# isteiakakis/Homomorphic-Encryption-Algorithms-Diploma-Thesis

Measured on AMD Instinct MI355X. Metric: CKKS matvec ciphertexts/sec (N=2^15, L=10), higher is better.
Workload: dtype u64; 1 GPU; he_linalg BatchedMatrix::matmul diag x col, 4096x4096 ct x ct matvec, N=2^15, L=10, default Galois keys; batch_per_gpu=128, n=4096, key_switches_per_matvec=18204, parallelism=replicated matrix+keys, dp1 over input vectors, batch_global=128

## Files before the change

### homomorphic-encryption-algorithms-diploma-thesis_amd/csrc/hec_engine.hip

```cpp
#include <algorithm>
#include <cmath>
#include <complex>
#include <cstdio>
#include <cstdlib>
#include <cstring>
#include <exception>
#include <limits>
#include <mutex>
#include <set>
#include <thread>
#include <tuple>

#include "hec_internal.h"

#include <dlfcn.h>
#include <unistd.h>
#include <rccl/rccl.h>
#include "hecdna.h"

using namespace hec;
using u128 = unsigned __int128;

struct HecComm {
    virtual ~HecComm() = default;
// ... 390 lines not shown
        fan_divide_round(c, ACC + l * N, 2 * (l + 1) * N, (l + 1) * N, Z, B * ng, 2, l, (int)c.K - 1);
    }
    for (int q = 0; q < ng; ++q) {
        ProfScope k(c, "k:k_ntt/divround_b", (6.0 + in_nk) * B * l);
        divide_round(c, ACC + q * sacc + l * N, 2 * (l + 1) * N, (l + 1) * N,
                     PolyArr{ACC + q * sacc, 2 * (l + 1) * N, (l + 1) * N}, IN, in_nk, OUT[q], B, 2, l, (int)c.K - 1,
                     c.p_inv.data(), c.p_inv_q.data(), Z + q * sz, elts[q], 2);
    }
}

void keyswitch(Ctx &c, Scratch &s, PolyArr T, const u64 *key, PolyArr IN, int in_nk, PolyArr OUT, int B, int l,
               u32 elt = 1)
{
    const u64 N = c.N;
    const std::size_t top = s.top;
    u64 *D = s.take(B * l * N), *E = s.take((u64)B * (l + 1) * l * N), *ACC = s.take((u64)B * 2 * (l + 1) * N),
        *Z = s.take((u64)B * 2 * l * N);
    int pmap[HEC_MAXL + 1];
    for (int i = 0; i <= HEC_MAXL; ++i) pmap[i] = i;
    const bool fan = c.fan_out && c.fused_modup_mac;
    const double K = l + 1;
    {
        ProfScope ps(c, "ks_intt");
        ProfScope k(c, fan ? "k:k_ntt/intt_b" : "k:k_ntt/intt2", 2.0 * B * l, fan ? 1 : 2);
        ntt_strided(c, true, T.p, T.sb, D, l * N, l, pmap, B * l, elt, fan ? 1 : 3);
    }
    if (c.fused_modup_mac) {
        {
            ProfScope ps(c, "ks_modup_a");
            ProfScope k(c, fan ? "k:k_fan2j/modup" : "k:k_ntt/modup_a", (double)B * l * (l + 1), 1);
            if (fan) fan_modup(c, D, E, B, l);
            else ks_modup_mac(c, D, E, T, key, ACC, B, l, 1, elt);
        }
        {
            ProfScope ps(c, "ks_bmac");
            ProfScope k(c, "k:k_bmac", (double)B * l * l + (double)B * l + 2.0 * l * K + 2.0 * B * K,
                        1);
            ks_modup_mac(c, D, E, T, key, ACC, B, l, 2, elt);
        }
    } else {
        {
            ProfScope ps(c, "ks_modup");
            ks_modup(c, D, E, B, l);
        }
        {
            ProfScope ps(c, "ks_mac");
            ks_mac(c, T, E, key, ACC, B, l, elt);
        }
    }
    moddown(c, ACC, Z, IN, in_nk, OUT, B, l, elt);
    s.top = top;
}

constexpr int HOIST_GROUP = 6;
struct Hoist {
    u64 *D = nullptr, *E = nullptr;
    int *zl = nullptr;
    u64 *acc0 = nullptr;
    u64 sacc = 0;
    u64 *acc(int q) const { return acc0 + (u64)q * sacc; }
};
std::size_t hoist_words(const Ctx &c, std::size_t B, std::size_t l)
{
    return c.N * B * (l + (l + 1) * l + (std::size_t)HOIST_GROUP * 2 * (l + 1)) +
           ((1 + B * l * (HEC_ZCAP + 1)) * sizeof(int) + 7) / 8 + 4 * 64;
}
// ... 818 lines not shown
        for (uint64_t i = 0; i < count; ++i) {
            need(bit_sizes[i] >= 2 && bit_sizes[i] <= 60, "bit_sizes is invalid");
            ++cnt[bit_sizes[i]];
        }
        const u64 factor = 2 * N;
        std::map<int, std::vector<u64>> table;
        for (auto &[b, k] : cnt) {
            u64 v = (((u64)1 << b) - 1) / factor * factor + 1;
            const u64 lo = (u64)1 << (b - 1);
            std::size_t left = k;
            while (left && v > lo) {
                if (isprime(v)) { table[b].push_back(v); --left; }
                v -= factor;
            }
            if (left) throw std::logic_error("failed to find enough qualifying primes");
        }
        for (uint64_t i = 0; i < count; ++i) {
            out[i] = table[bit_sizes[i]].back();
            table[bit_sizes[i]].pop_back();
        }
    });
}

int hec_context_create(uint64_t N, const uint64_t *mod, uint64_t K, int device, hec_context **out)
{
    return guard([&] {
        need(out != nullptr, "out is null");
        need(N >= 1024 && N <= 65536 && !(N & (N - 1)), "poly_modulus_degree must be a power of two in [2^10, 2^16]");
        need(K >= 2 && K - 1 <= HEC_MAXL, "coeff_modulus size is invalid");
        for (uint64_t i = 0; i < K; ++i)
            need(isprime(mod[i]) && (mod[i] - 1) % (2 * N) == 0 && !(mod[i] >> 60), "coeff_modulus is invalid");
        for (uint64_t i = 0; i < K; ++i)
            for (uint64_t j = 0; j < i; ++j) need(mod[i] != mod[j], "coeff_modulus is invalid");
        HEC_HIP(hipSetDevice(device));
        auto *ctx = new hec_context();
        Ctx &c = ctx->c;
        c.device = device;
        if (const char *f = std::getenv("HEC_FUSED_MODUP_MAC")) c.fused_modup_mac = f[0] != '0';
        if (const char *f = std::getenv("HEC_FUSE_GALOIS")) c.fuse_galois = f[0] != '0';
        if (const char *f = std::getenv("HEC_FAN")) c.fan_out = f[0] != '0';
        if (const char *f = std::getenv("HEC_HOIST_SCAN")) c.hoist_scan = std::atoi(f);
        if (const char *f = std::getenv("HEC_LANES")) c.lanes = std::max(1, std::atoi(f));
        if (const char *f = std::getenv("HEC_HOIST")) c.hoist = f[0] != '0';
        if (const char *f = std::getenv("HEC_HMAC")) c.hmac_cfg = std::atoi(f);
        if (const char *f = std::getenv("HEC_HMAC_ODD3")) c.hmac_odd3 = std::atoi(f);
        if (const char *f = std::getenv("HEC_HOIST_MIN")) c.hoist_min_children = std::max(1, std::atoi(f));
        if (const char *f = std::getenv("HEC_TENSOR_DEFER")) c.tensor_defer_max = std::max(1, std::atoi(f));
        if (const char *f = std::getenv("HEC_TENSOR_BUFS")) c.tensor_defer_bufs = std::max(1, std::atoi(f));
        if (const char *f = std::getenv("HEC_TENSOR_XCD")) c.tensor_xcd = std::max(0, std::atoi(f));
        if (const char *f = std::getenv("HEC_POISON")) c.poison = f[0] != '0';
        if (const char *f = std::getenv("HEC_LANE_SERIAL")) c.lane_serial = f[0] != '0';
        if (const char *f = std::getenv("HEC_DEBUG_LANES")) c.debug_lanes = f[0] != '0';
        if (const char *f = std::getenv("HEC_KERNEL_MEMOPS")) c.kernel_memops = f[0] != '0';
        if (const char *f = std::getenv("HEC_SPLIT_BFLY")) c.split_bfly = std::atoi(f);
        if (const char *f = std::getenv("HEC_NTTB_SHFL")) c.nttb_shfl = std::min(2, std::max(0, std::atoi(f)));
        if (const char *f = std::getenv("HEC_NTTB_SHFL_DR")) c.nttb_shfl_dr = std::atoi(f) != 0;
        if (const char *f = std::getenv("HEC_HMAC_INT")) c.hmac_int = std::atoi(f) != 0;
        if (const char *f = std::getenv("HEC_MODDOWN1")) c.moddown1 = std::atoi(f) != 0;
        if (const char *f = std::getenv("HEC_NT_E")) c.nt_e = std::atoi(f) != 0;
        if (const char *f = std::getenv("HEC_BMAC_SPLIT")) c.bmac_split = f[0] != '0';
        c.N = N;
        c.logN = __builtin_ctzll(N);
        c.K = K;
        c.L = K - 1;
        c.q.assign(mod, mod + K);
        for (u64 q : c.q) c.bits.push_back(64 - __builtin_clzll(q));
        HEC_HIP(hipStreamCreateWithFlags(&c.stream, hipStreamNonBlocking));
        c.own_stream = true;
        std::vector<ulonglong2> tw(K * N), itw(K * N);
        std::vector<u64> psipow(K * 2 * N);
// ... 46 lines not shown
            for (std::size_t k = 0; k < v.size(); ++k) r[k] = (double)v[k].x;
            return r;
        };
        const std::vector<double> twf = to_d(tw), itwf = to_d(itw), twbf = to_d(twb), itwbf = to_d(itwb);
        for (auto [dst, src] : {std::pair{&c.twf, &twf}, std::pair{&c.itwf, &itwf}, std::pair{&c.twbf, &twbf},
                                std::pair{&c.itwbf, &itwbf}}) {
            HEC_HIP(hipMalloc(dst, K * N * sizeof(double)));
            HEC_HIP(hipMemcpy(*dst, src->data(), K * N * sizeof(double), hipMemcpyHostToDevice));
        }
        HEC_HIP(hipMalloc(&c.twb, K * N * sizeof(ulonglong2)));
        HEC_HIP(hipMalloc(&c.itwb, K * N * sizeof(ulonglong2)));
        HEC_HIP(hipMemcpy(c.twb, twb.data(), K * N * sizeof(ulonglong2), hipMemcpyHostToDevice));
        HEC_HIP(hipMemcpy(c.itwb, itwb.data(), K * N * sizeof(ulonglong2), hipMemcpyHostToDevice));
        {
            std::vector<u64> tba(K * N, 0);
            for (uint64_t i = 0; i < K; ++i)
                if (!c.hprimes[i].fp)
                    for (uint64_t k = 0; k < N; ++k) tba[i * N + k] = (u64)(((u128)twb[i * N + k].x << 31) % c.q[i]);
            HEC_HIP(hipMalloc(&c.twbs, K * N * sizeof(u64)));
            HEC_HIP(hipMemcpy(c.twbs, tba.data(), K * N * sizeof(u64), hipMemcpyHostToDevice));
        }
        {
            HEC_HIP(hipMalloc(&c.psipow, psipow.size() * sizeof(u64)));
            HEC_HIP(hipMemcpy(c.psipow, psipow.data(), psipow.size() * sizeof(u64), hipMemcpyHostToDevice));
            std::vector<u64> cji(c.L * K);
            for (std::size_t J = 0; J < c.L; ++J)
                for (std::size_t I = 0; I < K; ++I) cji[J * K + I] = c.q[J] % c.q[I];
            HEC_HIP(hipMalloc(&c.cji, cji.size() * sizeof(u64)));
            HEC_HIP(hipMemcpy(c.cji, cji.data(), cji.size() * sizeof(u64), hipMemcpyHostToDevice));
            HEC_HIP(hipMalloc(&c.zflag, 2 * sizeof(int)));
            HEC_HIP(hipMemset(c.zflag, 0, 2 * sizeof(int)));
        }
        {
            std::vector<int> tab((c.L + 1) * (HEC_MAXL + 2), 0);
            c.imap_nint.assign(c.L + 1, 0);
            for (std::size_t l = 1; l <= c.L; ++l) {
                int *t = tab.data() + l * (HEC_MAXL + 2), n = 0;
                for (int pass = 0; pass < 2; ++pass)
                    for (int I = 0; I <= (int)l; ++I) {
                        const int kI = I == (int)l ? (int)K - 1 : I;
                        const bool fp = c.hprimes[kI].fp != 0;
                        if ((pass == 0) != fp) t[n++] = I;
                    }
                for (int I = 0; I <= (int)l; ++I)
                    if (!c.hprimes[I == (int)l ? K - 1 : I].fp) ++c.imap_nint[l];
            }
            HEC_HIP(hipMalloc(&c.imap, tab.size() * sizeof(int)));
            HEC_HIP(hipMemcpy(c.imap, tab.data(), tab.size() * sizeof(int), hipMemcpyHostToDevice));
        }
        HEC_HIP(hipMalloc(&c.primes, K * sizeof(DevPrime)));
        HEC_HIP(hipMemcpy(c.primes, c.hprimes.data(), K * sizeof(DevPrime), hipMemcpyHostToDevice));
        HEC_HIP(hipMalloc(&c.tw, K * N * sizeof(ulonglong2)));
        HEC_HIP(hipMalloc(&c.itw, K * N * sizeof(ulonglong2)));
        HEC_HIP(hipMemcpy(c.tw, tw.data(), K * N * sizeof(ulonglong2), hipMemcpyHostToDevice));
        HEC_HIP(hipMemcpy(c.itw, itw.data(), K * N * sizeof(ulonglong2), hipMemcpyHostToDevice));
        {
            std::vector<u64> ta(K * N, 0), ita(K * N, 0);
            for (uint64_t i = 0; i < K; ++i) {
                if (c.hprimes[i].fp) continue;
                const u64 q = c.q[i];
                for (uint64_t k = 0; k < N; ++k) {
                    ta[i * N + k] = (u64)(((u128)tw[i * N + k].x << 31) % q);
                    ita[i * N + k] = (u64)(((u128)itw[i * N + k].x << 31) % q);
                }
            }
            HEC_HIP(hipMalloc(&c.tws, K * N * sizeof(u64)));
            HEC_HIP(hipMalloc(&c.itws, K * N * sizeof(u64)));
            HEC_HIP(hipMemcpy(c.tws, ta.data(), K * N * sizeof(u64), hipMemcpyHostToDevice));
            HEC_HIP(hipMemcpy(c.itws, ita.data(), K * N * sizeof(u64), hipMemcpyHostToDevice));
        }
        const u64 P = c.q[K - 1];
        for (uint64_t i = 0; i < c.L; ++i) {
            const u64 q = c.q[i], pi = invm(P % q, q);
            c.p_inv.push_back(pi);
            c.p_inv_q.push_back(shoupq(pi, q));
// ... 60 lines not shown
            c.own_stream = false;
        } else {
            HEC_HIP(hipStreamCreateWithFlags(&c.stream, hipStreamNonBlocking));
            c.own_stream = true;
        }
    });
}

int hec_context_set_option(hec_context *ctx, const char *name, int64_t value)
{
    return guard([&] {
        need(ctx && name, "null argument");
        set_device(ctx);
        const std::string n(name);
        auto in = [&](int64_t lo, int64_t hi) {
            if (value < lo || value > hi)
                throw std::invalid_argument("option " + n + " takes " + std::to_string(lo) + ".." + std::to_string(hi));
            return (int)value;
        };
        auto apply = [&](Ctx &c) {
            if (n == "lanes") c.lanes = (int)std::max<int64_t>(1, value);
            else if (n == "lane_min_batch") c.lane_min_batch = (int)std::max<int64_t>(1, value);
            else if (n == "poison") c.poison = value != 0;
            else if (n == "lane_serial") c.lane_serial = value != 0;
            else if (n == "debug_lanes") c.debug_lanes = value != 0;
            else if (n == "kernel_memops") c.kernel_memops = value != 0;
            else if (n == "split_bfly") c.split_bfly = in(0, 4);
            else if (n == "nttb_shfl") c.nttb_shfl = in(0, 2);
            else if (n == "nttb_shfl_dr") c.nttb_shfl_dr = in(0, 1);
            else if (n == "hmac_int") c.hmac_int = in(0, 1);
            else if (n == "moddown1") c.moddown1 = in(0, 1);
            else if (n == "nt_e") c.nt_e = in(0, 1);
            else if (n == "bmac_split") c.bmac_split = value != 0;
            else if (n == "hoist") c.hoist = value != 0;
            else if (n == "hoist_min") c.hoist_min_children = (int)std::max<int64_t>(1, value);
            else if (n == "hmac") c.hmac_cfg = in(0, 2);
            else if (n == "hmac_odd3") c.hmac_odd3 = in(0, 1);
            else if (n == "hoist_scan") c.hoist_scan = in(0, 1);
            else if (n == "fan") c.fan_out = value != 0;
            else if (n == "fuse_galois") c.fuse_galois = value != 0;
            else if (n == "fused_modup_mac") c.fused_modup_mac = value != 0;
            else if (n == "tensor_defer") c.tensor_defer_max = (int)std::max<int64_t>(1, value);
            else if (n == "tensor_bufs") c.tensor_defer_bufs = (int)std::max<int64_t>(1, value);
            else if (n == "tensor_xcd") c.tensor_xcd = (int)std::max<int64_t>(0, value);
            else throw std::invalid_argument("unknown option");
        };
        HEC_HIP(hipStreamSynchronize(ctx->c.stream));
        apply(ctx->c);
        for (hec_context *l : ctx->lanes) {
            HEC_HIP(hipStreamSynchronize(l->c.stream));
            apply(l->c);
        }
    });
}

int hec_context_synchronize(hec_context *ctx)
{
    return guard([&] {
        set_device(ctx);
        HEC_HIP(hipStreamSynchronize(ctx->c.stream));
    });
}
uint64_t hec_context_poly_degree(const hec_context *ctx) { return ctx ? ctx->c.N : 0; }
uint64_t hec_context_key_moduli(const hec_context *ctx) { return ctx ? ctx->c.K : 0; }

uint32_t hec_galois_elt_from_step(const hec_context *ctx, int step)
// ... 1581 lines not shown
```

### homomorphic-encryption-algorithms-diploma-thesis_amd/csrc/hec_internal.h

```cpp
#pragma once
#include <hip/hip_runtime.h>

#include <cstdint>
#include <map>
#include <stdexcept>
#include <string>
#include <vector>

#include "hec_device.h"

namespace hec {

struct HipError : std::runtime_error {
    using std::runtime_error::runtime_error;
};
#define HEC_HIP(call)                                                                          \
    do {                                                                                       \
        hipError_t e_ = (call);                                                                \
        if (e_ != hipSuccess)                                                                  \
            throw ::hec::HipError(std::string(#call) + ": " + hipGetErrorString(e_));          \
    } while (0)

struct PolyArr {
    u64 *p = nullptr;
// ... 11 lines not shown
    void reserve(std::size_t w, hipStream_t stream);
    void reclaim(hipStream_t stream);
    void release();
};

struct Ctx {
    int device = 0;
    hipStream_t stream = nullptr;
    bool own_stream = false;
    std::size_t N = 0;
    int logN = 0;
    std::size_t K = 0, L = 0;
    std::vector<u64> q;
    std::vector<DevPrime> hprimes;
    std::vector<int> bits;
    DevPrime *primes = nullptr;
    ulonglong2 *tw = nullptr;
    ulonglong2 *itw = nullptr;
    ulonglong2 *twb = nullptr;
    ulonglong2 *itwb = nullptr;
    double *twf = nullptr, *itwf = nullptr, *twbf = nullptr, *itwbf = nullptr;
    u64 *tws = nullptr, *itws = nullptr;
    u64 *twbs = nullptr;
    bool bmac_split = true;
    int nttb_shfl = 0;
    int nt_e = 1;
    int moddown1 = 0;
    int hmac_int = 1;
    int nttb_shfl_dr = 0;
    int split_bfly = 4;
    int *imap = nullptr;
    std::vector<int> imap_nint;
    const int *imap_at(int l) const { return imap + (std::size_t)l * (HEC_MAXL + 2); }
    u64 *psipow = nullptr;
    u64 *cji = nullptr;
    int *zflag = nullptr;
    int logR = 0;
    u32 *enc_map = nullptr;
    double *enc_tw = nullptr;
    Workspace ws;
    std::vector<u64> p_inv, p_inv_q, p_half_mod;
    std::vector<std::vector<u64>> ql_inv, ql_inv_q, ql_half_mod;
    int tensor_defer_max = 12;
    int tensor_defer_bufs = 8;
    int tensor_xcd = 0;
    bool hoist = true;
    int hoist_min_children = 2;
    int hmac_cfg = 2;
    int hoist_scan = 1;
    int hmac_odd3 = 1;
    bool fan_out = true;
    int lanes = 1;
    int lane_min_batch = 16;
    bool fuse_galois = true;
    bool fused_modup_mac = true;
    bool poison = false;
    bool lane_serial = false;
    bool kernel_memops = true;
    bool debug_lanes = false;
    int prof_mode = 0;
    struct ProfRec { double ms = 0; uint64_t n = 0; double bytes = 0; uint64_t kl = 0; };
    std::map<std::string, ProfRec> prof_tab;
    struct ProfPend { const char *name; hipEvent_t e0, e1; double bytes; int kl; };
    std::vector<ProfPend> prof_pend;
    std::vector<hipEvent_t> ev_pool;
    std::size_t ev_used = 0;
    int total_bits(std::size_t level) const
    {
        int b = 0;
        for (std::size_t i = 0; i < level; ++i) b += bits[i];
        return b;
    }
};

void ntt_strided(Ctx &c, bool inverse, const u64 *src, u64 ps_src, u64 *dst, u64 ps_dst, int nl, const int *pmap,
                 int njobs, u32 elt = 1, int stages = 3);
void ks_modup(Ctx &c, const u64 *D, u64 *E, int B, int l, int stages = 3,
              bool mform = false);
void ks_mac(Ctx &c, PolyArr T, const u64 *E, const u64 *key, u64 *ACC, int B, int l, u32 elt);
void ks_modup_mac(Ctx &c, const u64 *D, u64 *E, PolyArr T, const u64 *key, u64 *ACC, int B, int l, int part,
                  u32 elt);
void divide_round(Ctx &c, const u64 *Y, u64 ysb, u64 ysk, PolyArr X, PolyArr IN, int in_nk, PolyArr OUT, int B,
                  int nk, int nl, int last_idx, const u64 *inv, const u64 *inv_q, u64 *Z, u32 in_elt = 1,
                  int stages = 3);
void fan_modup(Ctx &c, const u64 *D, u64 *E, int B, int l, bool direct = false, int *zl = nullptr);
#define HEC_ZCAP 8
void zero_scan(Ctx &c, const u64 *D, int nlimbs, int *zl);
void debug_count_zl(Ctx &c, const int *zl, int *cnt);
void dev_fill32(Ctx &c, void *p, u32 v, std::size_t bytes);
void dev_copy64(Ctx &c, u64 *dst, const u64 *src, std::size_t words);
void dev_fill(Ctx &c, void *p, u32 v, std::size_t bytes);
void dev_zero(Ctx &c, void *p, std::size_t bytes);
void hoisted_mac(Ctx &c, PolyArr X1, const u64 *E, const u64 *W, const int *zl, const u64 *key, u64 *ACC, int B,
                 int l, u32 elt);
struct HChildSpec {
    u32 elt, einv;
    const u64 *key, *W;
    u64 *ACC;
    const u64 *KW;
    const u64 *MK;
};
void mac_key_table(Ctx &c, const u64 *key, u64 *MK, u32 einv);
constexpr int HMAC_MAX_CHILDREN = 6;
void key_wsum(Ctx &c, const u64 *key, u64 *KW, int l);
void hoisted_mac_multi(Ctx &c, PolyArr X1, PolyArr X0, const u64 *E, const int *zl, const HChildSpec *kids, int nkids,
                       int B, int l);
void hoisted_mac_3(Ctx &c, PolyArr X1, PolyArr X0, const u64 *E, const int *zl, const HChildSpec *kids, int B, int l);
void hoisted_mac_group(Ctx &c, PolyArr X1, PolyArr X0, const u64 *E, const int *zl, const HChildSpec *kids, int nkids,
                       int B, int l);
int hoisted_group(const Ctx &c);
void fan_divide_round(Ctx &c, const u64 *Y, u64 ysb, u64 ysk, u64 *Z, int B, int nk, int nl, int last_idx);
bool moddown1(Ctx &c, const u64 *Y, u64 ysb, u64 ysk, PolyArr X, PolyArr IN, int in_nk, PolyArr OUT, int B, int nk,
              int nl, int last_idx, u32 elt);
void galois_permute(Ctx &c, PolyArr in, PolyArr out, int B, int nk, int nl, u32 elt);
// ... 28 lines not shown
```

### homomorphic-encryption-algorithms-diploma-thesis_amd/csrc/hec_kernels.hip

```cpp
#include "hec_internal.h"

#include <type_traits>

namespace hec {

typedef u64 u64x2 __attribute__((ext_vector_type(2)));
__device__ __forceinline__ ulonglong2 ld2(const u64 *p, u64 g)
{
    const u64x2 w = *reinterpret_cast<const u64x2 *>(p + g);
    return make_ulonglong2(w.x, w.y);
}
#ifndef HEC_NT_MASK
#define HEC_NT_MASK 0
#endif
constexpr int kNtMask = HEC_NT_MASK;
template <int BIT>
__device__ __forceinline__ void st1m(u64 *p, u64 v)
{
    if constexpr ((kNtMask & BIT) != 0) __builtin_nontemporal_store(v, p);
    else *p = v;
}
template <int BIT>
__device__ __forceinline__ void st2m(u64 *p, ulonglong2 v)
{
// ... 2447 lines not shown
    constexpr int LE = EPT == 16 ? 4 : EPT == 8 ? 3 : EPT == 4 ? 2 : 1;
    constexpr int D = S1 - S0, G = 1 << (LE - D), NQ = 1 << D;
    static_assert(D >= 1 && D <= LE, "round covers 1..log2(EPT) stages");
    constexpr bool PAIRS = TO_REG && S1 == LOGP;
#pragma unroll
    for (int gi = 0; gi < G; ++gi) {
        const int g = ts * G + gi;
        const int lo = g & ((1 << (LOGP - S1)) - 1);
        const int hi = g >> (LOGP - S1);
        const int xb = bswz<LOGP>((hi << (LOGP - S0)) | lo);
        GroupTw<S0, D, FP, !FP && HasSplitTw<TwG>::value> gt;
        gt.load(hi, twg);
        u64 v[NQ];
        if constexpr (PAIRS) {
#pragma unroll
            for (int a = 0; a < NQ; a += 2) {
                const ulonglong2 w = *(const ulonglong2 *)(row + (xb ^ bswz_c<LOGP>(a)));
                v[a] = w.x;
                v[a + 1] = w.y;
            }
        } else {
#pragma unroll
            for (int a = 0; a < NQ; ++a) v[a] = row[xb ^ bswz_c<LOGP>(a << (LOGP - S1))];
        }
        gt.template run<INV>(v, pr);
#pragma unroll
        for (int a = 0; a < NQ; ++a) {
            if constexpr (TO_REG) regs[gi * NQ + a] = v[a];
            else row[xb ^ bswz_c<LOGP>(a << (LOGP - S1))] = v[a];
        }
    }
}

template <int LOGP, int NSEG, int EPT, bool FP, bool SPL = false>
__device__ __forceinline__ void bmac_body(u64 *lds, u64 *ltw, u64 *ltwa, PolyArr T, const u64 *__restrict__ E,
                                          const u64 *__restrict__ key,
                                          u64 *__restrict__ ACC, const TwTables &tt, const DevPrime &pr, int I, int kI,
                                          int b, int xb, int logN, int l, int K, u32 elt)
{
    constexpr int P = 1 << LOGP, THREADS = NSEG * P / EPT, LD = bmac_ld(LOGP), TWS = 2 * P + 2;
    static_assert(BSwz<LOGP>::on || LOGP <= 6, "P = 128 / 256 chunk rows are swizzled: the padded rounds stop at P = 64");
    static_assert(BSwz<LOGP>::on == (LD == P), "bmac_ld must match the row layout");
    const u64 N = 1ull << logN;
    const int seg0 = xb * NSEG;
    const u64 base = (u64)seg0 << LOGP;
    const ulonglong2 *tw = tt.b + ((u64)kI << logN);
    const double *twf = tt.fb + ((u64)kI << logN);
    const u64 *twa = SPL ? tt.sb + ((u64)kI << logN) : nullptr;
    const int ts = (int)threadIdx.x % (P / EPT), sg = (int)threadIdx.x / (P / EPT);
    auto addr = [sg](int x) { return sg * LD + x + (x >> 4); };
    const u64 R = 1ull << (logN - LOGP);
    for (int t = threadIdx.x; t < NSEG * (P - 1); t += THREADS) {
        const int sl = t % NSEG, k = t / NSEG;
        const int st = 31 - __clz(k + 1), i = k + 1 - (1 << st);
        const u64 gi = R * ((1ull << st) - 1) + (u64)i * R + (u64)(seg0 + sl);
        if constexpr (FP) ltw[sl * TWS + k] = (u64)__double_as_longlong(twf[gi]);
        else {
            const ulonglong2 w = tw[gi];
            ltw[sl * TWS + 2 * k] = w.x;
            ltw[sl * TWS + 2 * k + 1] = w.y;
            if constexpr (SPL) ltwa[sl * P + k] = twa[gi];
        }
    }
    const LdsTw twg0{ltw + sg * TWS};
    const LdsTwS twgs{{ltw + sg * TWS}, ltwa + sg * P};
    const u64 g0 = ((u64)(seg0 + sg) << LOGP) + (u64)ts * EPT;
    auto src = [&](int J) -> const u64 * {
        return J == I ? T.p + b * T.sb + (u64)J * N : E + (((u64)((b * (l + 1) + I) * l + J)) << logN);
    };

    double f0[FP ? EPT : 1], f1[FP ? EPT : 1];
// ... 5 lines not shown
    }
    auto load_keys = [&](int J, u64 *k0, u64 *k1) {
        const u64 *kp0 = key + (((u64)(J * 2 + 0) * K + kI) << logN) + g0;
        const u64 *kp1 = key + (((u64)(J * 2 + 1) * K + kI) << logN) + g0;
#pragma unroll
        for (int e = 0; e < EPT; e += 2) {
            const ulonglong2 a = *(const ulonglong2 *)(kp0 + e), c = *(const ulonglong2 *)(kp1 + e);
            k0[e] = a.x; k0[e + 1] = a.y; k1[e] = c.x; k1[e + 1] = c.y;
        }
    };
    u64 nx[EPT];
    auto load_tile = [&](int J) {
        if (J == I && elt != 1) {
            const u64 *sp = src(J);
#pragma unroll
            for (int e = 0; e < EPT / 2; ++e) {
                const u32 t = galois_src((u32)(base + 2 * (threadIdx.x + e * THREADS)), elt, logN);
                const ulonglong2 w = *(const ulonglong2 *)(sp + (t & ~1u));
                nx[2 * e] = (t & 1) ? w.y : w.x;
                nx[2 * e + 1] = (t & 1) ? w.x : w.y;
            }
            return;
        }
        const ulonglong2 *sp = (const ulonglong2 *)(src(J) + base);
#pragma unroll
        for (int e = 0; e < EPT / 2; ++e) {
            const ulonglong2 w = sp[threadIdx.x + e * THREADS];
            nx[2 * e] = w.x;
            nx[2 * e + 1] = w.y;
        }
    };
    constexpr bool SWZ = BSwz<LOGP>::on;
    u64 *const row = lds + sg * LD;
    load_tile(0);
    for (int J = 0; J < l; ++J) {
        const bool ntt = J != I;
#pragma unroll
        for (int e = 0; e < EPT; e += 2) {
            const int li = 2 * (threadIdx.x + (e / 2) * THREADS);
            u64 v0 = nx[e], v1 = nx[e + 1];
            if constexpr (FP) {
                if (!ntt) {
                    v0 = (u64)__double_as_longlong(u2d(v0));
                    v1 = (u64)__double_as_longlong(u2d(v1));
                }
            }
            if constexpr (SWZ) {
                *(ulonglong2 *)(lds + (li / P) * LD + bswz<LOGP>(li % P)) = ulonglong2{v0, v1};
            } else {
                lds[(li / P) * LD + (li % P) + ((li % P) >> 4)] = v0;
                lds[(li / P) * LD + (li % P) + 1 + (((li % P) + 1) >> 4)] = v1;
            }
        }
        u64 k0[EPT], k1[EPT];
        load_keys(J, k0, k1);
        if (J + 1 < l) load_tile(J + 1);
        __syncthreads();
        u64 v[EPT];
        auto rounds = [&](const auto &twg) {
            static_assert(LOGP >= 5 && LOGP <= 8, "pass-B sizes 2^5 .. 2^8");
            static_assert(EPT == 4, "rounds of 2 stages");
            if constexpr (SWZ) {
                ntt_round_x<LOGP, 0, 2, EPT, false, FP, false>(row, ts, twg, pr, nullptr);
                __syncthreads();
                ntt_round_x<LOGP, 2, 4, EPT, false, FP, false>(row, ts, twg, pr, nullptr);
                __syncthreads();
                ntt_round_x<LOGP, 4, 6, EPT, false, FP, false>(row, ts, twg, pr, nullptr);
                __syncthreads();
                ntt_round_x<LOGP, 6, LOGP, EPT, false, FP, true>(row, ts, twg, pr, v);
            } else if constexpr (LOGP <= 6) {
                ntt_round_g<LOGP, 0, 2, EPT, false, FP, false>(lds, addr, ts, twg, pr, nullptr);
                __syncthreads();
                ntt_round_g<LOGP, 2, 4, EPT, false, FP, false>(lds, addr, ts, twg, pr, nullptr);
                __syncthreads();
                ntt_round_g<LOGP, 4, LOGP, EPT, false, FP, true>(lds, addr, ts, twg, pr, v);
            }
        };
        if (ntt) {
            if constexpr (!FP && SPL) rounds(twgs);
            else rounds(twg0);
        } else if constexpr (SWZ) {
            const int xb = bswz<LOGP>(ts * EPT);
#pragma unroll
            for (int e = 0; e < EPT; e += 2) {
                const ulonglong2 w = *(const ulonglong2 *)(row + (xb ^ bswz_c<LOGP>(e)));
                v[e] = w.x;
                v[e + 1] = w.y;
            }
        } else {
#pragma unroll
            for (int e = 0; e < EPT; ++e) v[e] = lds[addr(ts * EPT + e)];
        }
#pragma unroll
        for (int e = 0; e < EPT; ++e) {
            if constexpr (FP) {
                const double dv = __longlong_as_double((long long)v[e]);
                f0[e] += fp_mulmod(dv, u2d(k0[e]), pr.qd, pr.qinv);
                f1[e] += fp_mulmod(dv, u2d(k1[e]), pr.qd, pr.qinv);
            } else {
                mac128(i0[e], v[e], k0[e]);
                mac128(i1[e], v[e], k1[e]);
            }
        }
        __syncthreads();
    }
    u64 *o0 = ACC + (((u64)((b * 2 + 0) * (l + 1) + I)) << logN) + g0;
    u64 *o1 = ACC + (((u64)((b * 2 + 1) * (l + 1) + I)) << logN) + g0;
#pragma unroll
    for (int e = 0; e < EPT; e += 2) {
        if constexpr (FP) {
            *(ulonglong2 *)(o0 + e) = ulonglong2{fp_canon(f0[e], pr.qd, pr.qinv), fp_canon(f0[e + 1], pr.qd, pr.qinv)};
            *(ulonglong2 *)(o1 + e) = ulonglong2{fp_canon(f1[e], pr.qd, pr.qinv), fp_canon(f1[e + 1], pr.qd, pr.qinv)};
        } else {
            *(ulonglong2 *)(o0 + e) = ulonglong2{barrett128(i0[e].lo, i0[e].hi, pr.q, pr.r0, pr.r1),
                                                 barrett128(i0[e + 1].lo, i0[e + 1].hi, pr.q, pr.r0, pr.r1)};
            *(ulonglong2 *)(o1 + e) = ulonglong2{barrett128(i1[e].lo, i1[e].hi, pr.q, pr.r0, pr.r1),
                                                 barrett128(i1[e + 1].lo, i1[e + 1].hi, pr.q, pr.r0, pr.r1)};
        }
    }
}

template <int LOGP, int NSEG, int EPT, bool SPL>
__global__ void __launch_bounds__(NSEG *(1 << LOGP) / EPT, 4)
    k_bmac(PolyArr T, const u64 *__restrict__ E, const u64 *__restrict__ key, u64 *__restrict__ ACC, TwTables tt,
           const DevPrime *__restrict__ primes, const int *__restrict__ Imap, int nI, int logN, int l, int K,
           int nint, int gpad, u32 elt)
{
    __shared__ __attribute__((aligned(16))) u64 lds[NSEG * bmac_ld(LOGP)];
    __shared__ __attribute__((aligned(16))) u64 ltw[NSEG * (2 * (1 << LOGP) + 2)];
    __shared__ u64 ltwa[SPL ? NSEG * (1 << LOGP) : 1];
    const int w = blockIdx.x, B = gridDim.x / gpad;
    const int g8 = w & 7, rest = w >> 3, b = rest % B, G = (rest / B) * 8 + g8;
    const int X = (1 << (logN - LOGP)) / NSEG;
    if (G >= X * nI) return;
    const int yi = G / X, xb = G % X;
    const int I = Imap[yi];
    const int kI = I == l ? K - 1 : I;
    const DevPrime pr = primes[kI];
    if (yi < nint)
        bmac_body<LOGP, NSEG, EPT, false, SPL>(lds, ltw, ltwa, T, E, key, ACC, tt, pr, I, kI, b, xb, logN, l, K, elt);
    else
        bmac_body<LOGP, NSEG, EPT, true>(lds, ltw, ltwa, T, E, key, ACC, tt, pr, I, kI, b, xb, logN, l, K, elt);
}

template <int LOGR, int LOGC, int NA, int NB2, int EPT = 4>
static void run_modup_fused(Ctx &c, const u64 *D, u64 *E, PolyArr T, const u64 *key, u64 *ACC, int B, int l,
                            int part, u32 elt)
{
    constexpr int R = 1 << LOGR, C = 1 << LOGC;
    const TwTables fwd{c.tw, c.twb, c.twf, c.twbf, c.tws, c.twbs};
    const int nint = c.imap_nint[l];
    const int *dm = c.imap_at(l);
    if (part & 1) {
        ModUpMap m{l, c.logN, (int)c.K - 1};
        k_ntt<LOGR, NA, false, true, false><<<dim3(C / NA, B * l * l), NA * R / 16, 0, c.stream>>>(
            ModUpIO_A{m, D, E, c.primes}, fwd, c.primes, c.logN);
    }
    if (!(part & 2)) {
        HEC_HIP(hipGetLastError());
        return;
    }
    constexpr int TB = NB2 * C / EPT;
    constexpr int X = R / NB2;
    const int gpad = (X * (l + 1) + 7) / 8 * 8;
    if (c.bmac_split)
        k_bmac<LOGC, NB2, EPT, true><<<dim3(gpad * B), TB, 0, c.stream>>>(T, E, key, ACC, fwd, c.primes, dm, l + 1,
                                                                          c.logN, l, (int)c.K, nint, gpad, elt);
    else
        k_bmac<LOGC, NB2, EPT, false><<<dim3(gpad * B), TB, 0, c.stream>>>(T, E, key, ACC, fwd, c.primes, dm, l + 1,
                                                                           c.logN, l, (int)c.K, nint, gpad, elt);
    HEC_HIP(hipGetLastError());
}

void ks_modup_mac(Ctx &c, const u64 *D, u64 *E, PolyArr T, const u64 *key, u64 *ACC, int B, int l, int part,
                  u32 elt)
{
    switch (c.logN) {
    case 10: run_modup_fused<5, 5, 32, 16>(c, D, E, T, key, ACC, B, l, part, elt); break;
    case 11: run_modup_fused<6, 5, 32, 16>(c, D, E, T, key, ACC, B, l, part, elt); break;
    case 12: run_modup_fused<6, 6, 64, 8>(c, D, E, T, key, ACC, B, l, part, elt); break;
    case 13: run_modup_fused<7, 6, 32, 8>(c, D, E, T, key, ACC, B, l, part, elt); break;
    case 14: run_modup_fused<7, 7, 32, 4>(c, D, E, T, key, ACC, B, l, part, elt); break;
    case 15: run_modup_fused<8, 7, 16, 4>(c, D, E, T, key, ACC, B, l, part, elt); break;
    case 16: run_modup_fused<8, 8, 16, 4>(c, D, E, T, key, ACC, B, l, part, elt); break;
    default: throw std::invalid_argument("poly_modulus_degree must be 2^10 .. 2^16");
    }
}

template <int BT>
__device__ __forceinline__ void ks_mac_int(PolyArr T, const u64 *__restrict__ E, const u64 *__restrict__ key,
                                           u64 *__restrict__ ACC, int B, int l, int K, int logN,
                                           const DevPrime *__restrict__ primes, int I, u32 elt)
{
    const u64 N = 1ull << logN;
    const u64 g = (u64)blockIdx.x * 256 + threadIdx.x;
    const u64 tg = elt == 1 ? g : galois_src((u32)g, elt, logN);
    const int b0 = blockIdx.z * BT;
    const int kI = I == l ? K - 1 : I;
    const DevPrime pr = primes[kI];
    U128 a0[BT], a1[BT];
#pragma unroll
    for (int t = 0; t < BT; ++t) a0[t] = a1[t] = U128{0, 0};
    for (int J = 0; J < l; ++J) {
        const u64 k0 = key[((u64)(J * 2 + 0) * K + kI) * N + g];
        const u64 k1 = key[((u64)(J * 2 + 1) * K + kI) * N + g];
#pragma unroll
        for (int t = 0; t < BT; ++t) {
            const int b = b0 + t;
            if (b < B) {
                const u64 e = (I == J) ? T.p[b * T.sb + (u64)J * N + tg]
                                       : E[((u64)((b * (l + 1) + I) * l + J) << logN) + g];
                mac128(a0[t], e, k0);
                mac128(a1[t], e, k1);
            }
        }
    }
#pragma unroll
// ... 442 lines not shown
```

Measured before the change: 10.92 matvec/s.

## Fuse moddown divide-round into key-switch bmac kernel for Q primes

Splits the key-switch batched MAC into two launches. The special prime P is accumulated first, then inverse-NTT'd and converted via fan_divide_round. A second bmac launch over the Q primes then performs the moddown subtraction, scaling by P^-1 and the optional input add directly in its epilogue, instead of writing ACC and running a separate moddown pass. This is meant to remove a round trip of the Q-part accumulator through global memory and a separate kernel. In exchange it adds an extra NTT of Z in the bmac epilogue, more launches, and register pressure from the DR path. It is enabled by default except when moddown1 is set with logN=15.

```diff
diff --git a/homomorphic-encryption-algorithms-diploma-thesis_amd/csrc/hec_engine.hip b/homomorphic-encryption-algorithms-diploma-thesis_amd/csrc/hec_engine.hip
--- a/homomorphic-encryption-algorithms-diploma-thesis_amd/csrc/hec_engine.hip
+++ b/homomorphic-encryption-algorithms-diploma-thesis_amd/csrc/hec_engine.hip
@@ -446,6 +446,33 @@
             if (fan) fan_modup(c, D, E, B, l);
             else ks_modup_mac(c, D, E, T, key, ACC, B, l, 1, elt);
         }
+        if (fan && c.mac_divround && !(c.moddown1 && c.logN == 15)) {
+            const int pP[1] = {(int)c.K - 1};
+            {
+                ProfScope ps(c, "ks_bmac");
+                ProfScope k(c, "k:k_bmac/p", (double)B * l + 2.0 * l + 2.0 * B, 1);
+                ks_modup_mac(c, D, E, T, key, ACC, B, l, 2, elt, nullptr, 1);
+            }
+            {
+                ProfScope ps(c, "ks_moddown");
+                {
+                    ProfScope k(c, "k:k_ntt/moddown_intt", 4.0 * B, 1);
+                    ntt_strided(c, true, ACC + l * N, (l + 1) * N, ACC + l * N, (l + 1) * N, 1, pP, 2 * B, 1, 1);
+                }
+                ProfScope k(c, "k:k_fan2/moddown", 2.0 * B * (l + 1));
+                fan_divide_round(c, ACC + l * N, 2 * (l + 1) * N, (l + 1) * N, Z, B, 2, l, (int)c.K - 1);
+            }
+            {
+                ProfScope ps(c, "ks_bmac");
+                ProfScope k(c, "k:k_bmac/divround", (double)B * l * l + 2.0 * l * l + (4.0 + in_nk) * B * l, 1);
+                BmacDR dr{};
+                dr.Z = Z; dr.IN = IN; dr.OUT = OUT; dr.in_nk = in_nk;
+                for (int i = 0; i < l; ++i) { dr.inv[i] = c.p_inv[i]; dr.inv_q[i] = c.p_inv_q[i]; }
+                ks_modup_mac(c, D, E, T, key, ACC, B, l, 2, elt, &dr, 2);
+            }
+            s.top = top;
+            return;
+        }
         {
             ProfScope ps(c, "ks_bmac");
             ProfScope k(c, "k:k_bmac", (double)B * l * l + (double)B * l + 2.0 * l * K + 2.0 * B * K,
@@ -1330,10 +1357,18 @@
             need(isprime(mod[i]) && (mod[i] - 1) % (2 * N) == 0 && !(mod[i] >> 60), "coeff_modulus is invalid");
         for (uint64_t i = 0; i < K; ++i)
             for (uint64_t j = 0; j < i; ++j) need(mod[i] != mod[j], "coeff_modulus is invalid");
+        int mac_divround = -1;
+        if (const char *f = std::getenv("HEC_MAC_DIVROUND")) {
+            char *end = nullptr;
+            const long v = std::strtol(f, &end, 10);
+            need(end != f && *end == 0 && v >= 0 && v <= 1, "HEC_MAC_DIVROUND takes 0..1");
+            mac_divround = (int)v;
+        }
         HEC_HIP(hipSetDevice(device));
         auto *ctx = new hec_context();
         Ctx &c = ctx->c;
         c.device = device;
+        if (mac_divround >= 0) c.mac_divround = mac_divround;
         if (const char *f = std::getenv("HEC_FUSED_MODUP_MAC")) c.fused_modup_mac = f[0] != '0';
         if (const char *f = std::getenv("HEC_FUSE_GALOIS")) c.fuse_galois = f[0] != '0';
         if (const char *f = std::getenv("HEC_FAN")) c.fan_out = f[0] != '0';
@@ -1446,15 +1481,21 @@
             HEC_HIP(hipMemset(c.zflag, 0, 2 * sizeof(int)));
         }
         {
-            std::vector<int> tab((c.L + 1) * (HEC_MAXL + 2), 0);
+            std::vector<int> tab(2 * (c.L + 1) * (HEC_MAXL + 2), 0);
             c.imap_nint.assign(c.L + 1, 0);
+            c.imap_pint = c.hprimes[K - 1].fp ? 0 : 1;
             for (std::size_t l = 1; l <= c.L; ++l) {
                 int *t = tab.data() + l * (HEC_MAXL + 2), n = 0;
+                int *t2 = tab.data() + (c.L + 1 + l) * (HEC_MAXL + 2), n2 = 0;
+                t2[n2++] = (int)l;
                 for (int pass = 0; pass < 2; ++pass)
                     for (int I = 0; I <= (int)l; ++I) {
                         const int kI = I == (int)l ? (int)K - 1 : I;
                         const bool fp = c.hprimes[kI].fp != 0;
-                        if ((pass == 0) != fp) t[n++] = I;
+                        if ((pass == 0) != fp) {
+                            t[n++] = I;
+                            if (I != (int)l) t2[n2++] = I;
+                        }
                     }
                 for (int I = 0; I <= (int)l; ++I)
                     if (!c.hprimes[I == (int)l ? K - 1 : I].fp) ++c.imap_nint[l];
@@ -1581,6 +1622,7 @@
             else if (n == "moddown1") c.moddown1 = in(0, 1);
             else if (n == "nt_e") c.nt_e = in(0, 1);
             else if (n == "bmac_split") c.bmac_split = value != 0;
+            else if (n == "mac_divround") c.mac_divround = in(0, 1);
             else if (n == "hoist") c.hoist = value != 0;
             else if (n == "hoist_min") c.hoist_min_children = (int)std::max<int64_t>(1, value);
             else if (n == "hmac") c.hmac_cfg = in(0, 2);
diff --git a/homomorphic-encryption-algorithms-diploma-thesis_amd/csrc/hec_internal.h b/homomorphic-encryption-algorithms-diploma-thesis_amd/csrc/hec_internal.h
--- a/homomorphic-encryption-algorithms-diploma-thesis_amd/csrc/hec_internal.h
+++ b/homomorphic-encryption-algorithms-diploma-thesis_amd/csrc/hec_internal.h
@@ -67,6 +67,9 @@
     int *imap = nullptr;
     std::vector<int> imap_nint;
     const int *imap_at(int l) const { return imap + (std::size_t)l * (HEC_MAXL + 2); }
+    const int *imap_split_at(int l) const { return imap + (L + 1 + (std::size_t)l) * (HEC_MAXL + 2); }
+    int imap_pint = 0;
+    int mac_divround = 1;
     u64 *psipow = nullptr;
     u64 *cji = nullptr;
     int *zflag = nullptr;
@@ -113,8 +116,14 @@
 void ks_modup(Ctx &c, const u64 *D, u64 *E, int B, int l, int stages = 3,
               bool mform = false);
 void ks_mac(Ctx &c, PolyArr T, const u64 *E, const u64 *key, u64 *ACC, int B, int l, u32 elt);
+struct BmacDR {
+    const u64 *Z;
+    PolyArr IN, OUT;
+    int in_nk;
+    u64 inv[HEC_MAXL], inv_q[HEC_MAXL];
+};
 void ks_modup_mac(Ctx &c, const u64 *D, u64 *E, PolyArr T, const u64 *key, u64 *ACC, int B, int l, int part,
-                  u32 elt);
+                  u32 elt, const BmacDR *dr = nullptr, int tsel = 0);
 void divide_round(Ctx &c, const u64 *Y, u64 ysb, u64 ysk, PolyArr X, PolyArr IN, int in_nk, PolyArr OUT, int B,
                   int nk, int nl, int last_idx, const u64 *inv, const u64 *inv_q, u64 *Z, u32 in_elt = 1,
                   int stages = 3);
diff --git a/homomorphic-encryption-algorithms-diploma-thesis_amd/csrc/hec_kernels.hip b/homomorphic-encryption-algorithms-diploma-thesis_amd/csrc/hec_kernels.hip
--- a/homomorphic-encryption-algorithms-diploma-thesis_amd/csrc/hec_kernels.hip
+++ b/homomorphic-encryption-algorithms-diploma-thesis_amd/csrc/hec_kernels.hip
@@ -2503,11 +2503,17 @@
     }
 }
 
-template <int LOGP, int NSEG, int EPT, bool FP, bool SPL = false>
+struct BmacDRB {
+    const u64 *z[2], *in[2];
+    u64 *out[2];
+    u64 w, wq;
+};
+
+template <int LOGP, int NSEG, int EPT, bool FP, bool SPL = false, bool DR = false>
 __device__ __forceinline__ void bmac_body(u64 *lds, u64 *ltw, u64 *ltwa, PolyArr T, const u64 *__restrict__ E,
                                           const u64 *__restrict__ key,
                                           u64 *__restrict__ ACC, const TwTables &tt, const DevPrime &pr, int I, int kI,
-                                          int b, int xb, int logN, int l, int K, u32 elt)
+                                          int b, int xb, int logN, int l, int K, u32 elt, const BmacDRB &dr = BmacDRB{})
 {
     constexpr int P = 1 << LOGP, THREADS = NSEG * P / EPT, LD = bmac_ld(LOGP), TWS = 2 * P + 2;
     static_assert(BSwz<LOGP>::on || LOGP <= 6, "P = 128 / 256 chunk rows are swizzled: the padded rounds stop at P = 64");
@@ -2579,6 +2585,25 @@
     };
     constexpr bool SWZ = BSwz<LOGP>::on;
     u64 *const row = lds + sg * LD;
+    auto rounds = [&](const auto &twg, u64 *v) {
+        static_assert(LOGP >= 5 && LOGP <= 8, "pass-B sizes 2^5 .. 2^8");
+        static_assert(EPT == 4, "rounds of 2 stages");
+        if constexpr (SWZ) {
+            ntt_round_x<LOGP, 0, 2, EPT, false, FP, false>(row, ts, twg, pr, nullptr);
+            __syncthreads();
+            ntt_round_x<LOGP, 2, 4, EPT, false, FP, false>(row, ts, twg, pr, nullptr);
+            __syncthreads();
+            ntt_round_x<LOGP, 4, 6, EPT, false, FP, false>(row, ts, twg, pr, nullptr);
+            __syncthreads();
+            ntt_round_x<LOGP, 6, LOGP, EPT, false, FP, true>(row, ts, twg, pr, v);
+        } else if constexpr (LOGP <= 6) {
+            ntt_round_g<LOGP, 0, 2, EPT, false, FP, false>(lds, addr, ts, twg, pr, nullptr);
+            __syncthreads();
+            ntt_round_g<LOGP, 2, 4, EPT, false, FP, false>(lds, addr, ts, twg, pr, nullptr);
+            __syncthreads();
+            ntt_round_g<LOGP, 4, LOGP, EPT, false, FP, true>(lds, addr, ts, twg, pr, v);
+        }
+    };
     load_tile(0);
     for (int J = 0; J < l; ++J) {
         const bool ntt = J != I;
@@ -2604,28 +2629,9 @@
         if (J + 1 < l) load_tile(J + 1);
         __syncthreads();
         u64 v[EPT];
-        auto rounds = [&](const auto &twg) {
-            static_assert(LOGP >= 5 && LOGP <= 8, "pass-B sizes 2^5 .. 2^8");
-            static_assert(EPT == 4, "rounds of 2 stages");
-            if constexpr (SWZ) {
-                ntt_round_x<LOGP, 0, 2, EPT, false, FP, false>(row, ts, twg, pr, nullptr);
-                __syncthreads();
-                ntt_round_x<LOGP, 2, 4, EPT, false, FP, false>(row, ts, twg, pr, nullptr);
-                __syncthreads();
-                ntt_round_x<LOGP, 4, 6, EPT, false, FP, false>(row, ts, twg, pr, nullptr);
-                __syncthreads();
-                ntt_round_x<LOGP, 6, LOGP, EPT, false, FP, true>(row, ts, twg, pr, v);
-            } else if constexpr (LOGP <= 6) {
-                ntt_round_g<LOGP, 0, 2, EPT, false, FP, false>(lds, addr, ts, twg, pr, nullptr);
-                __syncthreads();
-                ntt_round_g<LOGP, 2, 4, EPT, false, FP, false>(lds, addr, ts, twg, pr, nullptr);
-                __syncthreads();
-                ntt_round_g<LOGP, 4, LOGP, EPT, false, FP, true>(lds, addr, ts, twg, pr, v);
-            }
-        };
         if (ntt) {
-            if constexpr (!FP && SPL) rounds(twgs);
-            else rounds(twg0);
+            if constexpr (!FP && SPL) rounds(twgs, v);
+            else rounds(twg0, v);
         } else if constexpr (SWZ) {
             const int xb = bswz<LOGP>(ts * EPT);
 #pragma unroll
@@ -2650,6 +2656,73 @@
             }
         }
         __syncthreads();
+    }
+    if constexpr (DR) {
+        const u64 two_q = 2 * pr.q;
+        auto load_z = [&](int k) {
+            const ulonglong2 *sp = (const ulonglong2 *)(dr.z[k] + base);
+#pragma unroll
+            for (int e = 0; e < EPT / 2; ++e) {
+                const ulonglong2 w = sp[threadIdx.x + e * THREADS];
+                nx[2 * e] = w.x;
+                nx[2 * e + 1] = w.y;
+            }
+        };
+        auto poly = [&](int k, auto *acc) {
+#pragma unroll
+            for (int e = 0; e < EPT; e += 2) {
+                const int li = 2 * (threadIdx.x + (e / 2) * THREADS);
+                if constexpr (SWZ) {
+                    *(ulonglong2 *)(lds + (li / P) * LD + bswz<LOGP>(li % P)) = ulonglong2{nx[e], nx[e + 1]};
+                } else {
+                    lds[(li / P) * LD + (li % P) + ((li % P) >> 4)] = nx[e];
+                    lds[(li / P) * LD + (li % P) + 1 + (((li % P) + 1) >> 4)] = nx[e + 1];
+                }
+            }
+            if (k == 0) load_z(1);
+            u64 in[EPT];
+            const u64 *ip = dr.in[k];
+            if (ip) {
+#pragma unroll
+                for (int e = 0; e < EPT; e += 2) {
+                    const u32 t = elt == 1 ? (u32)(g0 + e) : galois_src((u32)(g0 + e), elt, logN);
+                    const ulonglong2 w = *(const ulonglong2 *)(ip + (t & ~1u));
+                    in[e] = (t & 1) ? w.y : w.x;
+                    in[e + 1] = (t & 1) ? w.x : w.y;
+                }
+            }
+            __syncthreads();
+            u64 v[EPT];
+            if constexpr (!FP && SPL) rounds(twgs, v);
+            else rounds(twg0, v);
+            u64 r[EPT];
+#pragma unroll
+            for (int e = 0; e < EPT; ++e) {
+                if constexpr (FP) {
+                    const double x = fp_reduce(acc[e], pr.qd, pr.qinv);
+                    double y = fp_mulmod(x - __longlong_as_double((long long)v[e]), u2d(dr.w), pr.qd, pr.qinv);
+                    if (ip) y += u2d(in[e]);
+                    r[e] = fp_canon(y, pr.qd, pr.qinv);
+                } else {
+                    const u64 x = barrett128(acc[e].lo, acc[e].hi, pr.q, pr.r0, pr.r1);
+                    const u64 z = csub(csub(v[e], two_q), pr.q);
+                    r[e] = shoup(x + pr.q - z, dr.w, dr.wq, pr.q);
+                    if (ip) r[e] = addmod(r[e], in[e], pr.q);
+                }
+            }
+#pragma unroll
+            for (int e = 0; e < EPT; e += 2) st2m<2>(dr.out[k] + g0 + e, ulonglong2{r[e], r[e + 1]});
+            if (k == 0) __syncthreads();
+        };
+        load_z(0);
+        if constexpr (FP) {
+            poly(0, f0);
+            poly(1, f1);
+        } else {
+            poly(0, i0);
+            poly(1, i1);
+        }
+        return;
     }
     u64 *o0 = ACC + (((u64)((b * 2 + 0) * (l + 1) + I)) << logN) + g0;
     u64 *o1 = ACC + (((u64)((b * 2 + 1) * (l + 1) + I)) << logN) + g0;
@@ -2667,11 +2740,11 @@
     }
 }
 
-template <int LOGP, int NSEG, int EPT, bool SPL>
+template <int LOGP, int NSEG, int EPT, bool SPL, class... DRA>
 __global__ void __launch_bounds__(NSEG *(1 << LOGP) / EPT, 4)
     k_bmac(PolyArr T, const u64 *__restrict__ E, const u64 *__restrict__ key, u64 *__restrict__ ACC, TwTables tt,
            const DevPrime *__restrict__ primes, const int *__restrict__ Imap, int nI, int logN, int l, int K,
-           int nint, int gpad, u32 elt)
+           int nint, int gpad, u32 elt, const DRA... dra)
 {
     __shared__ __attribute__((aligned(16))) u64 lds[NSEG * bmac_ld(LOGP)];
     __shared__ __attribute__((aligned(16))) u64 ltw[NSEG * (2 * (1 << LOGP) + 2)];
@@ -2684,7 +2757,25 @@
     const int I = Imap[yi];
     const int kI = I == l ? K - 1 : I;
     const DevPrime pr = primes[kI];
-    if (yi < nint)
+    if constexpr (sizeof...(DRA) == 1) {
+        const BmacDR &d = (dra, ...);
+        BmacDRB db;
+#pragma unroll
+        for (int k = 0; k < 2; ++k) {
+            const u64 li = (u64)I << logN;
+            db.z[k] = d.Z + ((u64)((b * 2 + k) * l + I) << logN);
+            db.in[k] = (d.IN.p && k < d.in_nk) ? d.IN.p + b * d.IN.sb + k * d.IN.sk + li : nullptr;
+            db.out[k] = d.OUT.p + b * d.OUT.sb + k * d.OUT.sk + li;
+        }
+        db.w = d.inv[I];
+        db.wq = d.inv_q[I];
+        if (yi < nint)
+            bmac_body<LOGP, NSEG, EPT, false, SPL, true>(lds, ltw, ltwa, T, E, key, ACC, tt, pr, I, kI, b, xb, logN, l, K,
+                                                         elt, db);
+        else
+            bmac_body<LOGP, NSEG, EPT, true, false, true>(lds, ltw, ltwa, T, E, key, ACC, tt, pr, I, kI, b, xb, logN, l,
+                                                          K, elt, db);
+    } else if (yi < nint)
         bmac_body<LOGP, NSEG, EPT, false, SPL>(lds, ltw, ltwa, T, E, key, ACC, tt, pr, I, kI, b, xb, logN, l, K, elt);
     else
         bmac_body<LOGP, NSEG, EPT, true>(lds, ltw, ltwa, T, E, key, ACC, tt, pr, I, kI, b, xb, logN, l, K, elt);
@@ -2692,12 +2783,10 @@
 
 template <int LOGR, int LOGC, int NA, int NB2, int EPT = 4>
 static void run_modup_fused(Ctx &c, const u64 *D, u64 *E, PolyArr T, const u64 *key, u64 *ACC, int B, int l,
-                            int part, u32 elt)
+                            int part, u32 elt, const BmacDR *dr, int tsel)
 {
     constexpr int R = 1 << LOGR, C = 1 << LOGC;
     const TwTables fwd{c.tw, c.twb, c.twf, c.twbf, c.tws, c.twbs};
-    const int nint = c.imap_nint[l];
-    const int *dm = c.imap_at(l);
     if (part & 1) {
         ModUpMap m{l, c.logN, (int)c.K - 1};
         k_ntt<LOGR, NA, false, true, false><<<dim3(C / NA, B * l * l), NA * R / 16, 0, c.stream>>>(
@@ -2709,27 +2798,36 @@
     }
     constexpr int TB = NB2 * C / EPT;
     constexpr int X = R / NB2;
-    const int gpad = (X * (l + 1) + 7) / 8 * 8;
-    if (c.bmac_split)
-        k_bmac<LOGC, NB2, EPT, true><<<dim3(gpad * B), TB, 0, c.stream>>>(T, E, key, ACC, fwd, c.primes, dm, l + 1,
-                                                                          c.logN, l, (int)c.K, nint, gpad, elt);
-    else
-        k_bmac<LOGC, NB2, EPT, false><<<dim3(gpad * B), TB, 0, c.stream>>>(T, E, key, ACC, fwd, c.primes, dm, l + 1,
-                                                                           c.logN, l, (int)c.K, nint, gpad, elt);
+    const int *dm = tsel == 0 ? c.imap_at(l) : c.imap_split_at(l) + (tsel == 2 ? 1 : 0);
+    const int nI = tsel == 0 ? l + 1 : tsel == 1 ? 1 : l;
+    const int nint = tsel == 0 ? c.imap_nint[l] : tsel == 1 ? c.imap_pint : c.imap_nint[l] - c.imap_pint;
+    const int gpad = (X * nI + 7) / 8 * 8;
+    auto launch = [&](auto spl) {
+        constexpr bool SPL = decltype(spl)::value;
+        if (tsel == 2)
+            k_bmac<LOGC, NB2, EPT, SPL, BmacDR><<<dim3(gpad * B), TB, 0, c.stream>>>(
+                T, E, key, ACC, fwd, c.primes, dm, nI, c.logN, l, (int)c.K, nint, gpad, elt, *dr);
+        else
+            k_bmac<LOGC, NB2, EPT, SPL><<<dim3(gpad * B), TB, 0, c.stream>>>(T, E, key, ACC, fwd, c.primes, dm, nI,
+                                                                            c.logN, l, (int)c.K, nint, gpad, elt);
+    };
+    if (c.bmac_split) launch(std::true_type{});
+    else launch(std::false_type{});
     HEC_HIP(hipGetLastError());
 }
 
 void ks_modup_mac(Ctx &c, const u64 *D, u64 *E, PolyArr T, const u64 *key, u64 *ACC, int B, int l, int part,
-                  u32 elt)
-{
+                  u32 elt, const BmacDR *dr, int tsel)
+{
+    if ((tsel == 2) != (dr != nullptr) || tsel < 0 || tsel > 2) throw std::logic_error("ks_modup_mac: target selection");
     switch (c.logN) {
-    case 10: run_modup_fused<5, 5, 32, 16>(c, D, E, T, key, ACC, B, l, part, elt); break;
-    case 11: run_modup_fused<6, 5, 32, 16>(c, D, E, T, key, ACC, B, l, part, elt); break;
-    case 12: run_modup_fused<6, 6, 64, 8>(c, D, E, T, key, ACC, B, l, part, elt); break;
-    case 13: run_modup_fused<7, 6, 32, 8>(c, D, E, T, key, ACC, B, l, part, elt); break;
-    case 14: run_modup_fused<7, 7, 32, 4>(c, D, E, T, key, ACC, B, l, part, elt); break;
-    case 15: run_modup_fused<8, 7, 16, 4>(c, D, E, T, key, ACC, B, l, part, elt); break;
-    case 16: run_modup_fused<8, 8, 16, 4>(c, D, E, T, key, ACC, B, l, part, elt); break;
+    case 10: run_modup_fused<5, 5, 32, 16>(c, D, E, T, key, ACC, B, l, part, elt, dr, tsel); break;
+    case 11: run_modup_fused<6, 5, 32, 16>(c, D, E, T, key, ACC, B, l, part, elt, dr, tsel); break;
+    case 12: run_modup_fused<6, 6, 64, 8>(c, D, E, T, key, ACC, B, l, part, elt, dr, tsel); break;
+    case 13: run_modup_fused<7, 6, 32, 8>(c, D, E, T, key, ACC, B, l, part, elt, dr, tsel); break;
+    case 14: run_modup_fused<7, 7, 32, 4>(c, D, E, T, key, ACC, B, l, part, elt, dr, tsel); break;
+    case 15: run_modup_fused<8, 7, 16, 4>(c, D, E, T, key, ACC, B, l, part, elt, dr, tsel); break;
+    case 16: run_modup_fused<8, 8, 16, 4>(c, D, E, T, key, ACC, B, l, part, elt, dr, tsel); break;
     default: throw std::invalid_argument("poly_modulus_degree must be 2^10 .. 2^16");
     }
 }
```

New measurement: 11.05 matvec/s, median of 6. 1.3% higher.
